# gddickinson/neural_enhanced_super_resolution

Measured on AMD Instinct MI355X. Metric: output megapixels/sec, RealESRGAN_x2plus x2 upscale, higher is better.
Workload: dtype f32 (operands as f16 hi+lo pairs, 3 f16 MFMAs per product, f32 accumulate); 1 GPU; c2: 512x512->1024x1024 RealESRGAN_x2plus fp32 single tile; frames_in_flight_per_gpu=1, world_size=1, partition=independent frames, no data-path collective

## Files before the change

### neural_enhanced_super_resolution_amd/csrc/conv3x3_f16x2.hip

```cpp
#include <cstdlib>
#include <type_traits>

#include "f16x2_common.h"
#include "nesr_kernels.h"

namespace nesr {


namespace {

constexpr int TW = 32, PW = TW + 2;
constexpr int WAVES = 4;
constexpr int RW = 2;

template <int DMAW>
struct Geo {
    static constexpr int LAUNCH_THREADS = 64 * (WAVES + DMAW);
    static constexpr int THREADS = 64 * (DMAW ? DMAW : WAVES);
    static constexpr int TH = WAVES * RW;
    static constexpr int PH = TH + 2;
    static constexpr int NPIX = PH * PW;
    static constexpr int IN_ITEMS = 4 * NPIX;
    static constexpr int IN_ROUNDS = (IN_ITEMS + THREADS - 1) / THREADS;
    static constexpr int IN_BYTES = IN_ITEMS * 16;
// ... 226 lines not shown
            for (int e = 0; e < 16; ++e) sum += acc16[r][e & 1][(e >> 1) & 1][(e >> 2) & 1][e & 3];
        if (sum == 12345.678f) static_cast<float*>(a.out)[0] = sum;
        return;
    }

    const int cb = cb16;
    const uint16_t* res1 = static_cast<const uint16_t*>(a.res1);
    const uint16_t* res2 = static_cast<const uint16_t*>(a.res2);
    uint16_t* out = static_cast<uint16_t*>(a.out);
    uint16_t* out2 = static_cast<uint16_t*>(a.out2);
    bool bad = false;
    const bool poison = a.cout_real > 0 && a.status && __builtin_nontemporal_load(a.status) != 0u;
#pragma unroll
    for (int r = 0; r < RW; ++r)
#pragma unroll
        for (int nh = 0; nh < 2; ++nh) {
            const int Y = y0 + RW * wave + r, X = x0 + 16 * nh + j16;
            const bool valid = X < a.w_ && Y < y_hi;
            const size_t pix = ((size_t)n * a.h + (Y < a.h ? Y : 0)) * a.w_ + (X < a.w_ ? X : 0);
            f32x4 v0, v1;
#pragma unroll
            for (int i = 0; i < 4; ++i) {
                const float e = fmaf(acc16[r][nh][0][1][i], LO_INV, acc16[r][nh][0][0][i]);
                const float o = fmaf(acc16[r][nh][1][1][i], LO_INV, acc16[r][nh][1][0][i]);
                const auto sw_ = __builtin_amdgcn_permlane16_swap(__float_as_uint(e), __float_as_uint(o), false, false);
                v0[i] = __uint_as_float(sw_[0]);
                v1[i] = __uint_as_float(sw_[1]);
            }
            v0 += bz0;
            v1 += bz1;
            if (a.lrelu) {
#pragma unroll
                for (int i = 0; i < 4; ++i) { v0[i] = fmaxf(v0[i], v0[i] * 0.2f); v1[i] = fmaxf(v1[i], v1[i] * 0.2f); }
            }
            auto slot = [&](const Map& mp, int coff) -> size_t { return (size_t)((coff + 32 * cg) >> 4) * mp.chunk + pix * mp.pix + piece8; };
            if (res1) {
                f32x4 q0, q1;
                load_regrouped(res1 + slot(a.res1_map, 0), a.res1_map.chunk, q0, q1);
#pragma unroll
                for (int i = 0; i < 4; ++i) { v0[i] = __fadd_rn(__fmul_rn(v0[i], a.s1), q0[i]); v1[i] = __fadd_rn(__fmul_rn(v1[i], a.s1), q1[i]); }
            }
            if (res2) {
                f32x4 q0, q1;
                load_regrouped(res2 + slot(a.res2_map, 0), a.res2_map.chunk, q0, q1);
#pragma unroll
                for (int i = 0; i < 4; ++i) { v0[i] = __fadd_rn(__fmul_rn(v0[i], a.s2), q0[i]); v1[i] = __fadd_rn(__fmul_rn(v1[i], a.s2), q1[i]); }
            }
            if (out || out2) {
                uint4 cx, cx1;
                bool bad_here = false;
                split_regroup(v0, v1, cx, cx1, bad_here);
                bad |= bad_here && valid;
                if (valid && out) {
                    uint16_t* p = out + slot(a.out_map, a.out_coff);
                    store16(p, cx);
                    store16(p + a.out_map.chunk, cx1);
                }
                if (valid && out2) {
                    uint16_t* p = out2 + slot(a.out2_map, 0);
                    store16(p, cx);
                    store16(p + a.out2_map.chunk, cx1);
                }
            }
            if (!valid) continue;
            if (a.cout_real > 0 && cb == 0) {
#pragma unroll
                for (int q = 0; q < 4; ++q) {
                    if (q >= a.cout_real) break;
                    const float x = poison ? __builtin_nanf("") : v0[q];
                    if (a.out_nchw) a.out_nchw[(((size_t)n * a.cout_real + q) * a.h + Y) * a.w_ + X] = x;
                    if (a.out_u8) {
                        float qv = fminf(fmaxf(x, 0.f), 1.f) * 255.0f;
                        qv = a.u8_round ? rintf(qv) : truncf(qv);
                        const int ch = a.u8_flip ? (a.cout_real - 1 - q) : q;
                        a.out_u8[pix * a.cout_real + ch] = (uint8_t)qv;
                    }
                }
            }
        }
    if (bad && a.status) __hip_atomic_store(a.status, 1u, __ATOMIC_RELAXED, __HIP_MEMORY_SCOPE_AGENT);
    STAMP(3);
#if NESR_ABL & 64
    asm volatile("s_waitcnt vmcnt(0)" ::: "memory");
    STAMP(4);
#endif
}

struct RdbArgs {
    const void* cur;
    long long chunk_bytes;
    void* out;
    const void* res2;
    float s1, s2;
    const void* w[5];
    const float* bias[5];
    int n, h, w_;
    unsigned* progress;
    unsigned epoch;
    unsigned* abort_flag;
    unsigned* status;
    unsigned long long timeout_ticks;
};

__device__ __forceinline__ void glds16_s_sc1(const char* sbase, unsigned voff, unsigned lds_dst) {
    unsigned keep;
    asm volatile(
        "s_mov_b32 %0, m0\n\t"
        "s_mov_b32 m0, %3\n\t"
        "s_nop 0\n\t"
        "global_load_lds_dwordx4 %1, %2 sc1\n\t"
        "s_mov_b32 m0, %0"
        : "=&s"(keep)
        : "v"(voff), "s"(sbase), "s"(lds_dst)
        : "memory");
}
__device__ __forceinline__ void store16_wt_s(const char* sbase, unsigned voff, uint4 v) {
    asm volatile("global_store_dwordx4 %0, %1, %2 sc1\n\ts_nop 1" ::"v"(voff), "v"(__builtin_bit_cast(f32x4, v)), "s"(sbase) : "memory");
}

#ifndef NESR_RDB_ABL
#define NESR_RDB_ABL 0
#endif

__device__ __forceinline__ void wait_vmcnt_le(int k) {
    switch (k) {
        case 0: asm volatile("s_waitcnt vmcnt(0)" ::: "memory"); break;
        case 1: asm volatile("s_waitcnt vmcnt(1)" ::: "memory"); break;
        case 2: asm volatile("s_waitcnt vmcnt(2)" ::: "memory"); break;
        case 3: asm volatile("s_waitcnt vmcnt(3)" ::: "memory"); break;
        case 4: asm volatile("s_waitcnt vmcnt(4)" ::: "memory"); break;
        case 5: asm volatile("s_waitcnt vmcnt(5)" ::: "memory"); break;
        case 6: asm volatile("s_waitcnt vmcnt(6)" ::: "memory"); break;
        case 7: asm volatile("s_waitcnt vmcnt(7)" ::: "memory"); break;
        case 8: asm volatile("s_waitcnt vmcnt(8)" ::: "memory"); break;
        case 9: asm volatile("s_waitcnt vmcnt(9)" ::: "memory"); break;
        case 10: asm volatile("s_waitcnt vmcnt(10)" ::: "memory"); break;
        case 11: asm volatile("s_waitcnt vmcnt(11)" ::: "memory"); break;
        default: asm volatile("s_waitcnt vmcnt(12)" ::: "memory"); break;
    }
}

#if NESR_RDB_ABL & 256
__device__ unsigned long long g_rdb_stamps[2][64][8];
__device__ unsigned long long g_rdb_taps[2][8][8];
__device__ unsigned long long g_rdb_arrive[12][8][2];
#define RARRIVE(w, step, ev) do { if (blockIdx.x == 77 && lane == 0 && (step) >= 20 && (step) < 28) { unsigned long long t_ = __builtin_amdgcn_s_memtime(); asm volatile("s_waitcnt lgkmcnt(0)" ::: "memory"); g_rdb_arrive[w][(step) - 20][ev] = t_; } } while (0)
#define RSTAMP(role, step, ev) do { if (blockIdx.x == 77 && lane == 0) { unsigned long long t_ = __builtin_amdgcn_s_memtime(); asm volatile("s_waitcnt lgkmcnt(0)" ::: "memory"); g_rdb_stamps[role][step][ev] = t_; } } while (0)
#else
#define RSTAMP(role, step, ev) do { } while (0)
#define RARRIVE(w, step, ev) do { } while (0)
#endif

constexpr int RSLOTS = 4;
constexpr int MW = 8;
constexpr int DW = 4;
#ifndef NESR_RDB_PAR
#define NESR_RDB_PAR 0
#endif
#ifndef NESR_RDB_EPI_STEPS
#define NESR_RDB_EPI_STEPS 1
#endif
constexpr int EPI_STEPS = NESR_RDB_EPI_STEPS;
static_assert(EPI_STEPS <= 4 - (RSLOTS - 1), "the tile would wait for its own progress word");

__global__ __launch_bounds__(64 * (MW + DW), 3) void rdb_f16x2_kernel(RdbArgs a) {
    typedef Geo<4> G;
    constexpr int THREADS = G::THREADS, TH = G::TH;
    constexpr int IN_ITEMS = G::IN_ITEMS, IN_ROUNDS = G::IN_ROUNDS, IN_BYTES = G::IN_BYTES;
    constexpr int W_ROUNDS = (W_ITEMS + THREADS - 1) / THREADS;
    constexpr int WRING = RSLOTS * IN_BYTES;
    constexpr int BIAS = RSLOTS * (IN_BYTES + W_BYTES);
    static_assert(TH == MW, "one tile row per MFMA wave");
    extern __shared__ __attribute__((aligned(16))) char smem[];

    const int lane = threadIdx.x & 63;
    const int wave_all = __builtin_amdgcn_readfirstlane(threadIdx.x >> 6);
    const bool is_dma = wave_all >= MW;
    const bool is_cmp = !is_dma;
    const int wave = is_cmp ? wave_all : wave_all - MW;
    const int tid = wave * 64 + lane;

    const int tiles_x = (a.w_ + TW - 1) / TW;
    const int tiles_y = (a.h + TH - 1) / TH;
    const int total = tiles_x * tiles_y * a.n;
    int tile;
    {
        const int bid = blockIdx.x, q = total >> 3, r = total & 7, xcd = bid & 7;
        tile = (xcd < r ? xcd * (q + 1) : r * (q + 1) + (xcd - r) * q) + (bid >> 3);
    }
    const int n = tile / (tiles_x * tiles_y);
    const int t2 = tile - n * tiles_x * tiles_y;
    const int ty = t2 / tiles_x, tx = t2 - ty * tiles_x;
    const int y0 = ty * TH, x0 = tx * TW;

    const int j16 = lane & 15, g4 = lane >> 4;
    auto advance = [](int& l, int& cg, int& c) {
        const int nc = l == 4 ? 12 : 4 + 2 * l, ncg = l == 4 ? 2 : 1;
        if (++c == nc) { c = 0; if (++cg == ncg) { cg = 0; ++l; } }
    };

    if (is_dma) {
#ifdef NESR_RDB_DMAPRIO
        __builtin_amdgcn_s_setprio(NESR_RDB_DMAPRIO);
#endif
        const unsigned lds_base = (unsigned)(size_t)(lds_char*)(smem);
        unsigned voff[IN_ROUNDS];
        unsigned okmask = 0;
        unsigned wavemask = 0;
        const int row0 = y0 > 0 ? y0 - 1 : 0;
        const char* in_img = static_cast<const char*>(a.cur) + ((size_t)n * a.h + row0) * a.w_ * 64;
        const unsigned* watch = nullptr;
        int kdma = 0;
        if (lane < 9) {
            const int ny = ty + lane / 3 - 1, nx = tx + lane % 3 - 1;
            if (ny >= 0 && ny < tiles_y && nx >= 0 && nx < tiles_x) watch = a.progress + (n * tiles_y + ny) * tiles_x + nx;
        }
        {
            int p = tid >> 2;
            int py = p / PW, px = p - py * PW;
            const int sl = tid & 3;
#pragma unroll
            for (int i = 0; i < IN_ROUNDS; ++i) {
                const int k = tid + THREADS * i;
                const int sg = sl ^ (((px >> 2) & 1) << 1);
                const int Y = y0 - 1 + py, X = x0 - 1 + px;
                const bool has = k < IN_ITEMS;
                const bool ok = has && Y >= 0 && Y < a.h && X >= 0 && X < a.w_;
                voff[i] = ((unsigned)(Y - row0) * (unsigned)a.w_ + (unsigned)X) * 64u + sg * 16;
                okmask |= ok ? (1u << i) : 0u;
                if (__builtin_amdgcn_ballot_w64(ok) != 0ull) { wavemask |= 1u << i; ++kdma; }
                if (has && !ok) {
#pragma unroll
                    for (int sl2 = 0; sl2 < RSLOTS; ++sl2) *reinterpret_cast<f32x4*>(smem + sl2 * IN_BYTES + k * 16) = f32x4{0.f, 0.f, 0.f, 0.f};
                }
                px += (THREADS / 4) % PW;
                py += (THREADS / 4) / PW;
                if (px >= PW) { px -= PW; py += 1; }
            }
#pragma unroll
            for (int j = 0; j < W_ROUNDS; ++j) kdma += (wave * 64 + THREADS * j) < W_ITEMS ? 1 : 0;
        }
        unsigned seen = 0;
        bool gave_up = __hip_atomic_load(a.abort_flag, __ATOMIC_RELAXED, __HIP_MEMORY_SCOPE_AGENT) != 0u;
        auto dma_step = [&](int l, int cg, int c, int slot) {
            const int CG = l == 4 ? 2 : 1;
            const char* wsrc = static_cast<const char*>(a.w[l]) + ((size_t)c * CG + cg) * W_BYTES;
#pragma unroll
            for (int j = 0; j < W_ROUNDS; ++j) {
                const int k = tid + THREADS * j;
                const unsigned dst = lds_base + WRING + slot * W_BYTES + j * (THREADS * 16) + wave * 1024;
                if (k < W_ITEMS && !(NESR_RDB_ABL & 64)) glds16_s(wsrc, (unsigned)k * 16u, __builtin_amdgcn_readfirstlane(dst));
            }
            const unsigned need = c < 4 ? 0u : (unsigned)((c - 4) >> 1) + 1u;
            if (need > seen && !gave_up && !(NESR_RDB_ABL & 1)) {
                const unsigned target = a.epoch + need;
                unsigned long long t0 = 0;
                for (unsigned it = 0;; ++it) {
                    const unsigned v = watch ? __hip_atomic_load(watch, __ATOMIC_RELAXED, __HIP_MEMORY_SCOPE_AGENT) : target;
                    if (__builtin_amdgcn_ballot_w64((int)(v - target) < 0) == 0ull) break;
                    if ((it & 63u) == 0u) {
                        const unsigned long long now = __builtin_amdgcn_s_memrealtime();
                        if (it == 0) t0 = now;
                        const unsigned ab = __hip_atomic_load(a.abort_flag, __ATOMIC_RELAXED, __HIP_MEMORY_SCOPE_AGENT);
                        if (ab != 0u || now - t0 > a.timeout_ticks) {
                            if (ab == 0u && lane == 0) __hip_atomic_store(a.abort_flag, 1u | ((unsigned)c << 8) | ((unsigned)tile << 16), __ATOMIC_RELAXED, __HIP_MEMORY_SCOPE_AGENT);
                            gave_up = true;
                            break;
                        }
                    }
                    __builtin_amdgcn_s_sleep(4);
                }
                seen = need;
            }
            const char* isrc = in_img + (long long)c * a.chunk_bytes;
#pragma unroll
            for (int i = 0; i < IN_ROUNDS; ++i) {
                const unsigned dst = lds_base + slot * IN_BYTES + i * (THREADS * 16) + wave * 1024;
                if (((wavemask >> i) & 1u) && !(NESR_RDB_ABL & 32)) {
                    if ((okmask >> i) & 1u) {
                        if (NESR_RDB_ABL & 2) glds16_s(isrc, voff[i], __builtin_amdgcn_readfirstlane(dst));
                        else glds16_s_sc1(isrc, voff[i], __builtin_amdgcn_readfirstlane(dst));
                    }
                }
            }
        };
        if (wave == 0 && lane < 48) {
            const int l = lane >> 3 > 4 ? 4 : lane >> 3, cgq = lane >> 3 > 4 ? 8 + (lane & 7) : (lane & 7);
            *reinterpret_cast<f32x4*>(smem + BIAS + lane * 16) = *reinterpret_cast<const f32x4*>(a.bias[l] + 4 * cgq);
        }
        int fl = 0, fcg = 0, fc = 0;
        dma_step(0, 0, 0, 0);
        advance(fl, fcg, fc);
        dma_step(fl, fcg, fc, 1);
        advance(fl, fcg, fc);
        dma_step(fl, fcg, fc, 2);
        advance(fl, fcg, fc);
        asm volatile("s_waitcnt lgkmcnt(0)" ::: "memory");
        int fill = 3;
        int cl = 0, ccg = 0, cc = 0;
        wait_vmcnt_le((NESR_RDB_ABL & 96) ? 0 : 2 * kdma);
        __builtin_amdgcn_s_barrier();
        asm volatile("" ::: "memory");
        for (int step = 0; step < 52; ++step) {
            if (wave == 0) RSTAMP(1, step, 0);
#if NESR_RDB_ABL & 256
            if ((step == 0 || step == 51) && wave == 0 && blockIdx.x == 77 && lane == 0) {
                const unsigned long long r_ = __builtin_amdgcn_s_memrealtime(), t_ = __builtin_amdgcn_s_memtime();
                asm volatile("s_waitcnt lgkmcnt(0)" ::: "memory");
                g_rdb_stamps[1][step == 0 ? 62 : 63][0] = r_;
                g_rdb_stamps[1][step == 0 ? 62 : 63][1] = t_;
            }
#endif
            wait_vmcnt_le((step >= 50 || (NESR_RDB_ABL & 96)) ? 0 : kdma);
            if (wave == 0) RSTAMP(1, step, 1);
            RARRIVE(MW + wave, step, 0);
            if (!(NESR_RDB_ABL & 512)) __builtin_amdgcn_s_barrier();
            asm volatile("" ::: "memory");
            RARRIVE(MW + wave, step, 1);
            if (wave == 0) RSTAMP(1, step, 2);
            if (cc == EPI_STEPS && ccg == 0 && cl >= 1 && wave == 0 && lane == 0)
                __hip_atomic_store(a.progress + tile, a.epoch + (unsigned)cl, __ATOMIC_RELAXED, __HIP_MEMORY_SCOPE_AGENT);
            if (fl < 5) {
                dma_step(fl, fcg, fc, fill);
                advance(fl, fcg, fc);
                fill = fill == RSLOTS - 1 ? 0 : fill + 1;
            }
            if (wave == 0) RSTAMP(1, step, 3);
            advance(cl, ccg, cc);
        }
        return;
    }

#ifdef NESR_RDB_YPRIO
    if (wave >= 4) __builtin_amdgcn_s_setprio(NESR_RDB_YPRIO);
#endif
    const bool active = (y0 + wave) < a.h;
    const int un = g4 >> 1, kh = g4 & 1;
    int b16[5][2], a16[5];
#pragma unroll
    for (int st_ = 0; st_ < 5; ++st_) {
        const int dy = st_ < 3 ? un : 2;
        const int dx = st_ < 3 ? st_ : (st_ == 3 ? un : 2);
#pragma unroll
        for (int nh = 0; nh < 2; ++nh) {
            const int col = 16 * nh + j16 + dx;
            b16[st_][nh] = ((wave + dy) * PW + col) * 64 + ((kh ^ (((col >> 2) & 1) << 1)) << 4);
        }
        a16[st_] = ((((dy * 3 + dx) * 2) * 2 + kh) * 32 + j16) * 16;
    }
    int slot = 0;
#if NESR_RDB_ABL & 256
    int mstep = 0;
#endif
    typedef const __attribute__((address_space(3))) f32x4* lds_f32x4;
    const unsigned lds0 = (unsigned)(size_t)(lds_char*)(smem);
    unsigned bcur[5][2], acur[5], acur4b;
#pragma unroll
    for (int t = 0; t < 5; ++t) {
        bcur[t][0] = lds0 + (unsigned)b16[t][0];
        bcur[t][1] = lds0 + (unsigned)(t == 4 ? (b16[4][0] ^ ((un ^ 1) << 5)) : (b16[t][0] ^ 32));
        acur[t] = lds0 + (unsigned)(WRING + a16[t]);
    }
    acur4b = acur[4] + (unsigned)un * 1024u;
    const int par = (NESR_RDB_PAR >= 0) ? NESR_RDB_PAR : wave >> 2;
    const int cbl = (g4 & 1) * 16 + (g4 >> 1) * 8;
    const int piece8 = ((g4 & 1) * 2 + (g4 >> 1)) * 8;
    const bool res2 = a.res2 != nullptr;
    f32x4 ep[2][2];
#pragma unroll
    for (int nh = 0; nh < 2; ++nh)
#pragma unroll
        for (int mt = 0; mt < 2; ++mt) ep[nh][mt] = f32x4{0.f, 0.f, 0.f, 0.f};
    int ep_l = -1, ep_cg = 0;
    bool bad = false;
    auto unpack_res = [&](f32x4 rx, f32x4 rx1, f32x4& q0, f32x4& q1) {
        uint4 cx = __builtin_bit_cast(uint4, rx), cx1 = __builtin_bit_cast(uint4, rx1);
        regroup_pairs(cx, cx1);
        const f16x8 h = __builtin_bit_cast(f16x8, cx), lo = __builtin_bit_cast(f16x8, cx1);
#pragma unroll
        for (int i = 0; i < 4; ++i) {
            q0[i] = fmaf((float)lo[i], LO_INV, (float)h[i]);
            q1[i] = fmaf((float)lo[4 + i], LO_INV, (float)h[4 + i]);
        }
    };
    const long long row_bytes = (((long long)n * a.h + (y0 + wave)) * a.w_) * 64;
    unsigned lane_off[2];
    bool lane_ok[2];
#pragma unroll
    for (int nh = 0; nh < 2; ++nh) {
        const int X = x0 + 16 * nh + j16;
        lane_ok[nh] = X < a.w_;
        lane_off[nh] = (unsigned)(lane_ok[nh] ? X : 0) * 64u + (unsigned)piece8 * 2u;
    }
    auto uni = [](const char* p) -> const char* {
        const unsigned long long v = (unsigned long long)p;
        const unsigned lo = __builtin_amdgcn_readfirstlane((unsigned)v), hi = __builtin_amdgcn_readfirstlane((unsigned)(v >> 32));
        return (const char*)(((unsigned long long)hi << 32) | lo);
    };
    auto epi_half = [&](int l, int cg, const f32x4& e0, const f32x4& e1, int nh) {
#if NESR_RDB_ABL & 256
        if (wave == 1) RSTAMP(0, mstep, 3);
#endif
        const bool valid = lane_ok[nh];
        const unsigned voff = lane_off[nh];
        const char* bsrc = smem + BIAS + (l * 32 + 32 * cg + cbl) * 4;
        f32x4 v0, v1;
#pragma unroll
        for (int i = 0; i < 4; ++i) {
            const auto sw_ = __builtin_amdgcn_permlane16_swap(__float_as_uint(e0[i]), __float_as_uint(e1[i]), false, false);
            v0[i] = __uint_as_float(sw_[0]);
            v1[i] = __uint_as_float(sw_[1]);
        }
        v0 += *reinterpret_cast<const f32x4*>(bsrc);
        v1 += *reinterpret_cast<const f32x4*>(bsrc + 16);
        const int dchunk = l == 4 ? 2 * cg : 4 + 2 * l;
        if (l < 4) {
#pragma unroll
            for (int i = 0; i < 4; ++i) { v0[i] = fmaxf(v0[i], v0[i] * 0.2f); v1[i] = fmaxf(v1[i], v1[i] * 0.2f); }
        } else {
            const char* r1 = uni(static_cast<const char*>(a.cur) + (long long)(2 * cg) * a.chunk_bytes + row_bytes);
            const f32x4 r10 = *reinterpret_cast<const f32x4*>(r1 + voff), r11 = *reinterpret_cast<const f32x4*>(r1 + a.chunk_bytes + voff);
            f32x4 r20 = r10, r21 = r11;
            if (res2) {
                const char* r2 = uni(static_cast<const char*>(a.res2) + (long long)(2 * cg) * a.chunk_bytes + row_bytes);
                r20 = *reinterpret_cast<const f32x4*>(r2 + voff);
                r21 = *reinterpret_cast<const f32x4*>(r2 + a.chunk_bytes + voff);
            }
            f32x4 q0, q1;
            unpack_res(r10, r11, q0, q1);
#pragma unroll
            for (int i = 0; i < 4; ++i) { v0[i] = __fadd_rn(__fmul_rn(v0[i], a.s1), q0[i]); v1[i] = __fadd_rn(__fmul_rn(v1[i], a.s1), q1[i]); }
            if (res2) {
                unpack_res(r20, r21, q0, q1);
#pragma unroll
                for (int i = 0; i < 4; ++i) { v0[i] = __fadd_rn(__fmul_rn(v0[i], a.s2), q0[i]); v1[i] = __fadd_rn(__fmul_rn(v1[i], a.s2), q1[i]); }
            }
        }
#if NESR_RDB_ABL & 256
        asm volatile("" :: "v"(v0), "v"(v1));
        if (wave == 1) RSTAMP(0, mstep, 4);
#endif
        uint4 cx, cx1;
        bool bad_here = false;
        split_regroup(v0, v1, cx, cx1, bad_here);
        bad |= bad_here && valid;
#if NESR_RDB_ABL & 256
        asm volatile("" :: "v"(__builtin_bit_cast(f32x4, cx)), "v"(__builtin_bit_cast(f32x4, cx1)));
        if (wave == 1) RSTAMP(0, mstep, 5);
#endif
        if (valid) {
            const char* d0 = uni(static_cast<const char*>(l == 4 ? a.out : a.cur) + (long long)dchunk * a.chunk_bytes + row_bytes);
            if (l < 4 && !(NESR_RDB_ABL & 4)) {
                store16_wt_s(d0, voff, cx);
                store16_wt_s(d0 + a.chunk_bytes, voff, cx1);
            } else {
                *reinterpret_cast<uint4*>(const_cast<char*>(d0) + voff) = cx;
                *reinterpret_cast<uint4*>(const_cast<char*>(d0) + a.chunk_bytes + voff) = cx1;
            }
        }
#if NESR_RDB_ABL & 256
        if (wave == 1) RSTAMP(0, mstep, 6);
#endif
    };
    auto epi_part = [&](int c) {
        if (NESR_RDB_ABL & 16) return;
        if (EPI_STEPS == 1) {
            epi_half(ep_l, ep_cg, ep[0][0], ep[0][1], 0);
            epi_half(ep_l, ep_cg, ep[1][0], ep[1][1], 1);
        } else if (c == 0) {
            epi_half(ep_l, ep_cg, ep[0][0], ep[0][1], 0);
        } else {
            epi_half(ep_l, ep_cg, ep[1][0], ep[1][1], 1);
        }
    };
    f32x4 acc16[2][2][2];
    f32x4 Af[2][2][2];
    f32x4 Bf[2][2][2];
    auto load_step = [&](int sl, int s_, int buf) {
        const bool wrap = sl == RSLOTS - 1;
        const unsigned dB = wrap ? (unsigned)(-(RSLOTS - 1) * IN_BYTES) : (unsigned)IN_BYTES;
        const unsigned dA = wrap ? (unsigned)(-(RSLOTS - 1) * W_BYTES) : (unsigned)W_BYTES;
#pragma unroll
        for (int mt = 0; mt < 2; ++mt) {
            if (s_ < 4) {
                Af[buf][mt][0] = *((lds_f32x4)(size_t)(acur[s_] + mt * 256));
                Af[buf][mt][1] = *((lds_f32x4)(size_t)(acur[s_] + mt * 256 + 1024));
            } else {
                f32x4 hi = *((lds_f32x4)(size_t)(acur[4] + mt * 256));
                Af[buf][mt][1] = *((lds_f32x4)(size_t)(acur4b + mt * 256));
                if (un) hi = f32x4{0.f, 0.f, 0.f, 0.f};
                Af[buf][mt][0] = hi;
            }
        }
#pragma unroll
        for (int nh = 0; nh < 2; ++nh) {
            Bf[buf][nh][0] = *((lds_f32x4)(size_t)(bcur[s_][0] + nh * 1024));
            Bf[buf][nh][1] = *((lds_f32x4)(size_t)(bcur[s_][1] + nh * 1024));
        }
        acur[s_] += dA;
        if (s_ == 4) acur4b += dA;
        bcur[s_][0] += dB;
        bcur[s_][1] += dB;
    };
    auto step_body = [&](auto Pc, int c, bool last_of_all) {
        constexpr int P = decltype(Pc)::value;
        if (c == EPI_STEPS) asm volatile("s_waitcnt vmcnt(0)" ::: "memory");
#if NESR_RDB_ABL & 256
        if (wave == 1) RSTAMP(0, mstep, 0);
        RARRIVE(wave, mstep, 0);
#endif
        if (!(NESR_RDB_ABL & 512)) __builtin_amdgcn_s_barrier();
        asm volatile("" ::: "memory");
#if NESR_RDB_ABL & 256
        RARRIVE(wave, mstep, 1);
        if (wave == 1) RSTAMP(0, mstep, 1);
#endif
        const bool epi_now = active && ep_l >= 0 && c < EPI_STEPS;
        const int nslot = slot == RSLOTS - 1 ? 0 : slot + 1;
        if (active && !(NESR_RDB_ABL & 8)) {
            if (epi_now && par == 0) {
                epi_part(c);
                __builtin_amdgcn_sched_barrier(0);
            }
#if NESR_RDB_ABL & 256
            unsigned long long tt[6];
#endif
#pragma unroll
            for (int s_ = 0; s_ < 5; ++s_) {
                const int buf = (s_ + P) & 1;
#if NESR_RDB_ABL & 256
                tt[s_] = __builtin_amdgcn_s_memtime();
                __builtin_amdgcn_sched_barrier(0);
#endif
                if (s_ + 1 < 5) load_step(slot, s_ + 1, buf ^ 1);
                else if (!last_of_all) load_step(nslot, 0, buf ^ 1);
#pragma unroll
                for (int mt = 0; mt < 2; ++mt) {
                    const f16x8 a0 = __builtin_bit_cast(f16x8, Af[buf][mt][0]), a1 = __builtin_bit_cast(f16x8, Af[buf][mt][1]);
#pragma unroll
                    for (int nh = 0; nh < 2; ++nh) {
                        const f16x8 x0_ = __builtin_bit_cast(f16x8, Bf[buf][nh][0]), x1_ = __builtin_bit_cast(f16x8, Bf[buf][nh][1]);
                        if (s_ < 4) {
                            acc16[nh][mt][1] = __builtin_amdgcn_mfma_f32_16x16x32_f16(a0, x1_, acc16[nh][mt][1], 0, 0, 0);
                            acc16[nh][mt][0] = __builtin_amdgcn_mfma_f32_16x16x32_f16(a0, x0_, acc16[nh][mt][0], 0, 0, 0);
                            acc16[nh][mt][1] = __builtin_amdgcn_mfma_f32_16x16x32_f16(a1, x0_, acc16[nh][mt][1], 0, 0, 0);
                        } else {
                            acc16[nh][mt][0] = __builtin_amdgcn_mfma_f32_16x16x32_f16(a0, x0_, acc16[nh][mt][0], 0, 0, 0);
                            acc16[nh][mt][1] = __builtin_amdgcn_mfma_f32_16x16x32_f16(a1, x1_, acc16[nh][mt][1], 0, 0, 0);
                        }
                    }
                }
#pragma unroll
                for (int i = 0; i < 8; ++i) {
                    __builtin_amdgcn_sched_group_barrier(0x008, 1, 0);
                    __builtin_amdgcn_sched_group_barrier(0x100, 1, 0);
                }
                __builtin_amdgcn_sched_barrier(0);
            }
            if (epi_now && par == 1) {
                epi_part(c);
                __builtin_amdgcn_sched_barrier(0);
            }
#if NESR_RDB_ABL & 256
            tt[5] = __builtin_amdgcn_s_memtime();
            if (blockIdx.x == 77 && (wave == 1 || wave == 5) && lane == 0 && mstep >= 20 && mstep < 28) {
#pragma unroll
                for (int i = 0; i < 6; ++i) g_rdb_taps[wave == 5][mstep - 20][i] = tt[i];
            }
#endif
        }
        slot = nslot;
#if NESR_RDB_ABL & 256
        if (wave == 1) RSTAMP(0, mstep, 2);
        ++mstep;
#endif
    };
    __builtin_amdgcn_s_barrier();
    asm volatile("" ::: "memory");
    if (active) load_step(0, 0, 0);
    for (int l = 0; l < 5; ++l) {
        const int nc = l == 4 ? 12 : 4 + 2 * l;
        const int ncg = l == 4 ? 2 : 1;
        for (int cg = 0; cg < ncg; ++cg) {
#pragma unroll
            for (int nh = 0; nh < 2; ++nh)
#pragma unroll
                for (int mt = 0; mt < 2; ++mt)
#pragma unroll
                    for (int q = 0; q < 2; ++q) acc16[nh][mt][q] = f32x4{0.f, 0.f, 0.f, 0.f};
            for (int c = 0; c < nc; c += 2) {
                step_body(std::integral_constant<int, 0>{}, c, false);
                step_body(std::integral_constant<int, 1>{}, c + 1, l == 4 && cg == 1 && c + 2 == nc);
            }
#pragma unroll
            for (int nh = 0; nh < 2; ++nh)
#pragma unroll
                for (int mt = 0; mt < 2; ++mt)
#pragma unroll
                    for (int i = 0; i < 4; ++i) ep[nh][mt][i] = fmaf(acc16[nh][mt][1][i], LO_INV, acc16[nh][mt][0][i]);
            ep_l = l;
            ep_cg = cg;
        }
    }
    if (active && !(NESR_RDB_ABL & 16)) {
        epi_half(4, 1, ep[0][0], ep[0][1], 0);
        epi_half(4, 1, ep[1][0], ep[1][1], 1);
    }
    if (bad && a.status) __hip_atomic_store(a.status, 1u, __ATOMIC_RELAXED, __HIP_MEMORY_SCOPE_AGENT);
}

template <int DMAW, int NMT = 2>
hipError_t launch_split(const ConvArgs& a, hipStream_t s) {
    typedef Geo<DMAW> G;
    constexpr size_t shm = (size_t)ISLOTS * G::IN_BYTES + 2 * (size_t)W_BYTES;
    static unsigned long long attr_done = 0;
    {
        const hipError_t e = ensure_dynamic_lds(reinterpret_cast<const void*>(&conv3x3_f16x2_kernel<DMAW, NMT>), shm, attr_done);
        if (e != hipSuccess) return e;
    }
    const int rows = (a.y_hi > 0 ? a.y_hi : a.h) - a.y_lo;
    const long total = (long)((a.w_ + TW - 1) / TW) * ((rows + G::TH - 1) / G::TH) * a.n * (a.coutp / 32);
    if (total <= 0) return hipSuccess;
    if (total > 0x7fffffffL) return hipErrorInvalidValue;
    hipLaunchKernelGGL((conv3x3_f16x2_kernel<DMAW, NMT>), dim3((unsigned)total), dim3(G::LAUNCH_THREADS), shm, s, a);
    return hipGetLastError();
}


}

#if NESR_RDB_ABL & 256
extern "C" int nesr_debug_rdb_stamps(unsigned long long* out) {
    return (int)hipMemcpyFromSymbol(out, HIP_SYMBOL(g_rdb_stamps), sizeof(unsigned long long) * 2 * 64 * 8);
}
extern "C" int nesr_debug_rdb_taps(unsigned long long* out) {
    return (int)hipMemcpyFromSymbol(out, HIP_SYMBOL(g_rdb_taps), sizeof(unsigned long long) * 2 * 8 * 8);
}
extern "C" int nesr_debug_rdb_arrive(unsigned long long* out) {
    return (int)hipMemcpyFromSymbol(out, HIP_SYMBOL(g_rdb_arrive), sizeof(unsigned long long) * 12 * 8 * 2);
}
#endif
#if NESR_ABL & 64
extern "C" int nesr_debug_stamps(unsigned long long* out, int n) {
    return (int)hipMemcpyFromSymbol(out, HIP_SYMBOL(g_stamps), sizeof(unsigned long long) * (n < 256 ? n : 256));
}
#endif

size_t packed_weight_elems_f16x2(int cin_p, int coutp) { return (size_t)cin_p * 9 * coutp * 2; }

void pack_weights_f16x2(const float* oihw, int cout, int cin, int cin_p, int coutp, uint16_t* dst) {
    const size_t total = packed_weight_elems_f16x2(cin_p, coutp);
    for (size_t i = 0; i < total; ++i) dst[i] = 0;
    const int groups = coutp / 32;
    for (int o = 0; o < cout; ++o)
        for (int ci = 0; ci < cin; ++ci)
            for (int tap = 0; tap < 9; ++tap) {
                const float wv = oihw[((size_t)o * cin + ci) * 9 + tap];
                const uint16_t hi = f2h(wv);
                const uint16_t lo = f2h((wv - h2f(hi)) * LO_SCALE);
                const int c = ci / 16, kh = (ci % 16) / 8, kk = ci % 8;
                const size_t slab = ((size_t)c * groups + o / 32) * (size_t)(W_ITEMS * 8);
                const size_t ihi = slab + ((((size_t)tap * 2 + 0) * 2 + kh) * 32 + o % 32) * 8 + kk;
                const size_t ilo = slab + ((((size_t)tap * 2 + 1) * 2 + kh) * 32 + o % 32) * 8 + kk;
                dst[ihi] = hi;
                dst[ilo] = lo;
            }
}

int rdb_f16x2_tiles(int n, int h, int w) { return ((w + TW - 1) / TW) * ((h + 7) / 8) * n; }

hipError_t launch_rdb_f16x2(const RdbLaunch& r, hipStream_t s) {
    typedef Geo<4> G;
    constexpr size_t shm = (size_t)RSLOTS * (G::IN_BYTES + (size_t)W_BYTES) + 768;
    static unsigned long long attr_done = 0;
    {
        const hipError_t e = ensure_dynamic_lds(reinterpret_cast<const void*>(&rdb_f16x2_kernel), shm, attr_done);
        if (e != hipSuccess) return e;
    }
    if ((long long)r.w_ * 64 * 12 >= (1ll << 32)) return hipErrorInvalidValue;
    RdbArgs a;
    a.cur = r.cur; a.chunk_bytes = r.chunk_bytes; a.out = r.out; a.res2 = r.res2; a.s1 = r.s1; a.s2 = r.s2;
    for (int i = 0; i < 5; ++i) { a.w[i] = r.w[i]; a.bias[i] = r.bias[i]; }
    a.n = r.n; a.h = r.h; a.w_ = r.w_;
    a.progress = r.progress; a.epoch = r.epoch; a.abort_flag = r.abort_flag; a.status = r.status;
    a.timeout_ticks = r.timeout_ticks ? r.timeout_ticks : 20000000ull;
    int total = rdb_f16x2_tiles(r.n, r.h, r.w_);
    if (total <= 0) return hipSuccess;
    static int resident = -1;
    if (resident < 0) {
        int per_cu = 0, dev = 0, cus = 0;
        if (hipOccupancyMaxActiveBlocksPerMultiprocessor(&per_cu, rdb_f16x2_kernel, 64 * (MW + DW), shm) != hipSuccess || hipGetDevice(&dev) != hipSuccess ||
            hipDeviceGetAttribute(&cus, hipDeviceAttributeMultiprocessorCount, dev) != hipSuccess)
            return hipErrorUnknown;
        resident = per_cu * cus;
    }
    if (total > resident) return hipErrorLaunchOutOfResources;
    total -= r.debug_drop;
    if (total <= 0) return hipSuccess;
    hipLaunchKernelGGL(rdb_f16x2_kernel, dim3((unsigned)total), dim3(64 * (MW + DW)), shm, s, a);
    return hipGetLastError();
}

hipError_t launch_conv3x3_f16x2(const ConvArgs& a, hipStream_t s) {
    if (a.cin % 16 || (a.coutp != 32 && a.coutp != 64)) return hipErrorInvalidValue;
    if (a.y_lo < 0 || (a.y_hi > 0 && (a.y_hi > a.h || a.y_hi <= a.y_lo)) || (a.y_hi == 0 && a.y_lo != 0)) return hipErrorInvalidValue;
    if ((long long)a.in_w * 64 * 12 >= (1ll << 32)) return hipErrorInvalidValue;
    if (a.in_map.pix != 32 || (a.out && (a.out_map.pix % 32 || a.out_coff % 16))) return hipErrorInvalidValue;
    if ((a.out_nchw || a.out_u8) && (a.coutp != 32 || a.cout_real < 1 || a.cout_real > 4)) return hipErrorInvalidValue;
    static const int cus = [] {
        int dev = 0, n = 256;
        if (hipGetDevice(&dev) != hipSuccess || hipDeviceGetAttribute(&n, hipDeviceAttributeMultiprocessorCount, dev) != hipSuccess) n = 256;
        return n;
    }();
    static const int dmaw = [] { const char* e = getenv("NESR_SPLIT_DMAW"); return e ? atoi(e) : -1; }();
    const long t1 = (long)((a.w_ + TW - 1) / TW) * (((a.y_hi > 0 ? a.y_hi : a.h) - a.y_lo + 7) / 8) * a.n * (a.coutp >> 5);
    const bool producer = dmaw >= 0 ? dmaw > 0 : (t1 <= cus && !a.shared_device);
    if (a.narrow_last && (a.out_nchw || a.out_u8) && !a.out && !a.out2 && !a.res1 && !a.res2)
        return producer ? launch_split<4, 1>(a, s) : launch_split<0, 1>(a, s);
    return producer ? launch_split<4>(a, s) : launch_split<0>(a, s);
}

}
```

Baseline: 159.7 MP/s.

## Fuse conv5's two output-channel groups into one pass over shared input slabs

Inside the fused RDB kernel, the fifth conv no longer runs its two 32-channel output groups as separate sweeps. Each input slab is now loaded once and feeds two accumulator sets, so the conv5 steps go from 24 to 12. The weight DMA is split from the input DMA: conv5 weight pairs are streamed into ring positions 0,1 / 2,3, and the vmcnt wait tracks the real number of in-flight loads. This removes half the input LDS reads and DMA steps for conv5, but doubles the accumulator registers, which may lower occupancy or cause spills under launch bounds of 3.

Result: faster. 168.4 MP/s (median of 6 runs) (+5.5%).

```diff
diff --git a/neural_enhanced_super_resolution_amd/csrc/conv3x3_f16x2.hip b/neural_enhanced_super_resolution_amd/csrc/conv3x3_f16x2.hip
--- a/neural_enhanced_super_resolution_amd/csrc/conv3x3_f16x2.hip
+++ b/neural_enhanced_super_resolution_amd/csrc/conv3x3_f16x2.hip
@@ -402,6 +402,10 @@
 #endif
 
 constexpr int RSLOTS = 4;
+constexpr int RDB_STEP5 = 4 + 6 + 8 + 10;
+constexpr int RDB_STEPS = RDB_STEP5 + 12;
+constexpr int W5_ROUNDS = 2 * W_ITEMS / (64 * 4);
+static_assert(RSLOTS == 4 && RDB_STEP5 % RSLOTS == 0 && W5_ROUNDS * 64 * 4 == 2 * W_ITEMS, "conv5's slab pairs sit at ring positions 0,1 / 2,3 and fill whole DMA rounds");
 constexpr int MW = 8;
 constexpr int DW = 4;
 #ifndef NESR_RDB_PAR
@@ -444,9 +448,9 @@
     const int y0 = ty * TH, x0 = tx * TW;
 
     const int j16 = lane & 15, g4 = lane >> 4;
-    auto advance = [](int& l, int& cg, int& c) {
-        const int nc = l == 4 ? 12 : 4 + 2 * l, ncg = l == 4 ? 2 : 1;
-        if (++c == nc) { c = 0; if (++cg == ncg) { cg = 0; ++l; } }
+    auto advance = [](int& l, int& c) {
+        const int nc = l == 4 ? 12 : 4 + 2 * l;
+        if (++c == nc) { c = 0; ++l; }
     };
 
     if (is_dma) {
@@ -460,7 +464,7 @@
         const int row0 = y0 > 0 ? y0 - 1 : 0;
         const char* in_img = static_cast<const char*>(a.cur) + ((size_t)n * a.h + row0) * a.w_ * 64;
         const unsigned* watch = nullptr;
-        int kdma = 0;
+        int kin = 0, kw = 0;
         if (lane < 9) {
             const int ny = ty + lane / 3 - 1, nx = tx + lane % 3 - 1;
             if (ny >= 0 && ny < tiles_y && nx >= 0 && nx < tiles_x) watch = a.progress + (n * tiles_y + ny) * tiles_x + nx;
@@ -478,7 +482,7 @@
                 const bool ok = has && Y >= 0 && Y < a.h && X >= 0 && X < a.w_;
                 voff[i] = ((unsigned)(Y - row0) * (unsigned)a.w_ + (unsigned)X) * 64u + sg * 16;
                 okmask |= ok ? (1u << i) : 0u;
-                if (__builtin_amdgcn_ballot_w64(ok) != 0ull) { wavemask |= 1u << i; ++kdma; }
+                if (__builtin_amdgcn_ballot_w64(ok) != 0ull) { wavemask |= 1u << i; ++kin; }
                 if (has && !ok) {
 #pragma unroll
                     for (int sl2 = 0; sl2 < RSLOTS; ++sl2) *reinterpret_cast<f32x4*>(smem + sl2 * IN_BYTES + k * 16) = f32x4{0.f, 0.f, 0.f, 0.f};
@@ -488,19 +492,28 @@
                 if (px >= PW) { px -= PW; py += 1; }
             }
 #pragma unroll
-            for (int j = 0; j < W_ROUNDS; ++j) kdma += (wave * 64 + THREADS * j) < W_ITEMS ? 1 : 0;
+            for (int j = 0; j < W_ROUNDS; ++j) kw += (wave * 64 + THREADS * j) < W_ITEMS ? 1 : 0;
         }
         unsigned seen = 0;
         bool gave_up = __hip_atomic_load(a.abort_flag, __ATOMIC_RELAXED, __HIP_MEMORY_SCOPE_AGENT) != 0u;
-        auto dma_step = [&](int l, int cg, int c, int slot) {
-            const int CG = l == 4 ? 2 : 1;
-            const char* wsrc = static_cast<const char*>(a.w[l]) + ((size_t)c * CG + cg) * W_BYTES;
+        auto dma_w = [&](int l, int c, int wpos) {
+            const char* wsrc = static_cast<const char*>(a.w[l]) + (size_t)c * W_BYTES;
 #pragma unroll
             for (int j = 0; j < W_ROUNDS; ++j) {
                 const int k = tid + THREADS * j;
-                const unsigned dst = lds_base + WRING + slot * W_BYTES + j * (THREADS * 16) + wave * 1024;
+                const unsigned dst = lds_base + WRING + wpos * W_BYTES + j * (THREADS * 16) + wave * 1024;
                 if (k < W_ITEMS && !(NESR_RDB_ABL & 64)) glds16_s(wsrc, (unsigned)k * 16u, __builtin_amdgcn_readfirstlane(dst));
             }
+        };
+        auto dma_w5 = [&](int c, int wpos) {
+            const char* wsrc = static_cast<const char*>(a.w[4]) + (size_t)c * (2 * W_BYTES);
+#pragma unroll
+            for (int j = 0; j < W5_ROUNDS; ++j) {
+                const unsigned dst = lds_base + WRING + wpos * W_BYTES + j * (THREADS * 16) + wave * 1024;
+                if (!(NESR_RDB_ABL & 64)) glds16_s(wsrc, (unsigned)(tid + THREADS * j) * 16u, __builtin_amdgcn_readfirstlane(dst));
+            }
+        };
+        auto dma_in = [&](int c, int slot) {
             const unsigned need = c < 4 ? 0u : (unsigned)((c - 4) >> 1) + 1u;
             if (need > seen && !gave_up && !(NESR_RDB_ABL & 1)) {
                 const unsigned target = a.epoch + need;
@@ -538,45 +551,54 @@
             const int l = lane >> 3 > 4 ? 4 : lane >> 3, cgq = lane >> 3 > 4 ? 8 + (lane & 7) : (lane & 7);
             *reinterpret_cast<f32x4*>(smem + BIAS + lane * 16) = *reinterpret_cast<const f32x4*>(a.bias[l] + 4 * cgq);
         }
-        int fl = 0, fcg = 0, fc = 0;
-        dma_step(0, 0, 0, 0);
-        advance(fl, fcg, fc);
-        dma_step(fl, fcg, fc, 1);
-        advance(fl, fcg, fc);
-        dma_step(fl, fcg, fc, 2);
-        advance(fl, fcg, fc);
+        int fl = 0, fc = 0;
+#pragma unroll
+        for (int i = 0; i < RSLOTS - 1; ++i) {
+            dma_w(0, i, i);
+            dma_in(i, i);
+            advance(fl, fc);
+        }
         asm volatile("s_waitcnt lgkmcnt(0)" ::: "memory");
         int fill = 3;
-        int cl = 0, ccg = 0, cc = 0;
-        wait_vmcnt_le((NESR_RDB_ABL & 96) ? 0 : 2 * kdma);
+        int cl = 0, cc = 0;
+        wait_vmcnt_le((NESR_RDB_ABL & 96) ? 0 : 2 * (kw + kin));
+        int inflight = kw + kin;
         __builtin_amdgcn_s_barrier();
         asm volatile("" ::: "memory");
-        for (int step = 0; step < 52; ++step) {
+        for (int step = 0; step < RDB_STEPS; ++step) {
             if (wave == 0) RSTAMP(1, step, 0);
 #if NESR_RDB_ABL & 256
-            if ((step == 0 || step == 51) && wave == 0 && blockIdx.x == 77 && lane == 0) {
+            if ((step == 0 || step == RDB_STEPS - 1) && wave == 0 && blockIdx.x == 77 && lane == 0) {
                 const unsigned long long r_ = __builtin_amdgcn_s_memrealtime(), t_ = __builtin_amdgcn_s_memtime();
                 asm volatile("s_waitcnt lgkmcnt(0)" ::: "memory");
                 g_rdb_stamps[1][step == 0 ? 62 : 63][0] = r_;
                 g_rdb_stamps[1][step == 0 ? 62 : 63][1] = t_;
             }
 #endif
-            wait_vmcnt_le((step >= 50 || (NESR_RDB_ABL & 96)) ? 0 : kdma);
+            wait_vmcnt_le((NESR_RDB_ABL & 96) ? 0 : inflight);
             if (wave == 0) RSTAMP(1, step, 1);
             RARRIVE(MW + wave, step, 0);
             if (!(NESR_RDB_ABL & 512)) __builtin_amdgcn_s_barrier();
             asm volatile("" ::: "memory");
             RARRIVE(MW + wave, step, 1);
             if (wave == 0) RSTAMP(1, step, 2);
-            if (cc == EPI_STEPS && ccg == 0 && cl >= 1 && wave == 0 && lane == 0)
+            if (cc == EPI_STEPS && cl >= 1 && wave == 0 && lane == 0)
                 __hip_atomic_store(a.progress + tile, a.epoch + (unsigned)cl, __ATOMIC_RELAXED, __HIP_MEMORY_SCOPE_AGENT);
+            inflight = 0;
+            if (step + 1 >= RDB_STEP5) {
+                if (step + 1 < RDB_STEPS) dma_w5(step + 1 - RDB_STEP5, ((step + 1) & 1) * 2);
+            } else if (fl < 4) {
+                dma_w(fl, fc, (step + RSLOTS - 1) & (RSLOTS - 1));
+                inflight += kw;
+            }
             if (fl < 5) {
-                dma_step(fl, fcg, fc, fill);
-                advance(fl, fcg, fc);
+                dma_in(fc, fill);
+                inflight += kin;
+                advance(fl, fc);
                 fill = fill == RSLOTS - 1 ? 0 : fill + 1;
             }
             if (wave == 0) RSTAMP(1, step, 3);
-            advance(cl, ccg, cc);
+            advance(cl, cc);
         }
         return;
     }
@@ -599,19 +621,20 @@
         a16[st_] = ((((dy * 3 + dx) * 2) * 2 + kh) * 32 + j16) * 16;
     }
     int slot = 0;
+    int wpos = 0;
 #if NESR_RDB_ABL & 256
     int mstep = 0;
 #endif
     typedef const __attribute__((address_space(3))) f32x4* lds_f32x4;
     const unsigned lds0 = (unsigned)(size_t)(lds_char*)(smem);
-    unsigned bcur[5][2], acur[5], acur4b;
-#pragma unroll
-    for (int t = 0; t < 5; ++t) {
-        bcur[t][0] = lds0 + (unsigned)b16[t][0];
-        bcur[t][1] = lds0 + (unsigned)(t == 4 ? (b16[4][0] ^ ((un ^ 1) << 5)) : (b16[t][0] ^ 32));
-        acur[t] = lds0 + (unsigned)(WRING + a16[t]);
-    }
-    acur4b = acur[4] + (unsigned)un * 1024u;
+    unsigned bcur[5], aw012, aw3, aw4, aw4b;
+#pragma unroll
+    for (int t = 0; t < 5; ++t) bcur[t] = lds0 + (unsigned)b16[t][0];
+    const unsigned xl4 = (unsigned)((un ^ 1) << 5);
+    aw012 = lds0 + (unsigned)(WRING + a16[0]);
+    aw3 = lds0 + (unsigned)(WRING + a16[3]);
+    aw4 = lds0 + (unsigned)(WRING + a16[4]);
+    aw4b = aw4 + (unsigned)un * 1024u;
     const int par = (NESR_RDB_PAR >= 0) ? NESR_RDB_PAR : wave >> 2;
     const int cbl = (g4 & 1) * 16 + (g4 >> 1) * 8;
     const int piece8 = ((g4 & 1) * 2 + (g4 >> 1)) * 8;
@@ -621,7 +644,7 @@
     for (int nh = 0; nh < 2; ++nh)
 #pragma unroll
         for (int mt = 0; mt < 2; ++mt) ep[nh][mt] = f32x4{0.f, 0.f, 0.f, 0.f};
-    int ep_l = -1, ep_cg = 0;
+    int ep_l = -1;
     bool bad = false;
     auto unpack_res = [&](f32x4 rx, f32x4 rx1, f32x4& q0, f32x4& q1) {
         uint4 cx = __builtin_bit_cast(uint4, rx), cx1 = __builtin_bit_cast(uint4, rx1);
@@ -715,44 +738,75 @@
     auto epi_part = [&](int c) {
         if (NESR_RDB_ABL & 16) return;
         if (EPI_STEPS == 1) {
-            epi_half(ep_l, ep_cg, ep[0][0], ep[0][1], 0);
-            epi_half(ep_l, ep_cg, ep[1][0], ep[1][1], 1);
+            epi_half(ep_l, 0, ep[0][0], ep[0][1], 0);
+            epi_half(ep_l, 0, ep[1][0], ep[1][1], 1);
         } else if (c == 0) {
-            epi_half(ep_l, ep_cg, ep[0][0], ep[0][1], 0);
+            epi_half(ep_l, 0, ep[0][0], ep[0][1], 0);
         } else {
-            epi_half(ep_l, ep_cg, ep[1][0], ep[1][1], 1);
-        }
-    };
-    f32x4 acc16[2][2][2];
+            epi_half(ep_l, 0, ep[1][0], ep[1][1], 1);
+        }
+    };
+    f32x4 acc16[2][2][2][2];
     f32x4 Af[2][2][2];
     f32x4 Bf[2][2][2];
-    auto load_step = [&](int sl, int s_, int buf) {
-        const bool wrap = sl == RSLOTS - 1;
-        const unsigned dB = wrap ? (unsigned)(-(RSLOTS - 1) * IN_BYTES) : (unsigned)IN_BYTES;
-        const unsigned dA = wrap ? (unsigned)(-(RSLOTS - 1) * W_BYTES) : (unsigned)W_BYTES;
+    auto load_a = [&](int s_, int buf, unsigned off) {
 #pragma unroll
         for (int mt = 0; mt < 2; ++mt) {
             if (s_ < 4) {
-                Af[buf][mt][0] = *((lds_f32x4)(size_t)(acur[s_] + mt * 256));
-                Af[buf][mt][1] = *((lds_f32x4)(size_t)(acur[s_] + mt * 256 + 1024));
+                const unsigned ad = s_ < 3 ? aw012 + s_ * 2048 : aw3;
+                Af[buf][mt][0] = *((lds_f32x4)(size_t)(ad + off + mt * 256));
+                Af[buf][mt][1] = *((lds_f32x4)(size_t)(ad + off + mt * 256 + 1024));
             } else {
-                f32x4 hi = *((lds_f32x4)(size_t)(acur[4] + mt * 256));
-                Af[buf][mt][1] = *((lds_f32x4)(size_t)(acur4b + mt * 256));
+                f32x4 hi = *((lds_f32x4)(size_t)(aw4 + off + mt * 256));
+                Af[buf][mt][1] = *((lds_f32x4)(size_t)(aw4b + off + mt * 256));
                 if (un) hi = f32x4{0.f, 0.f, 0.f, 0.f};
                 Af[buf][mt][0] = hi;
             }
         }
+    };
+    auto move_a = [&](unsigned d) {
+        aw012 += d;
+        aw3 += d;
+        aw4 += d;
+        aw4b += d;
+    };
+    auto load_b = [&](int sl, int s_, int buf) {
+        const unsigned dB = sl == RSLOTS - 1 ? (unsigned)(-(RSLOTS - 1) * IN_BYTES) : (unsigned)IN_BYTES;
+        const unsigned xl = bcur[s_] ^ (s_ == 4 ? xl4 : 32u);
 #pragma unroll
         for (int nh = 0; nh < 2; ++nh) {
-            Bf[buf][nh][0] = *((lds_f32x4)(size_t)(bcur[s_][0] + nh * 1024));
-            Bf[buf][nh][1] = *((lds_f32x4)(size_t)(bcur[s_][1] + nh * 1024));
-        }
-        acur[s_] += dA;
-        if (s_ == 4) acur4b += dA;
-        bcur[s_][0] += dB;
-        bcur[s_][1] += dB;
-    };
-    auto step_body = [&](auto Pc, int c, bool last_of_all) {
+            Bf[buf][nh][0] = *((lds_f32x4)(size_t)(bcur[s_] + nh * 1024));
+            Bf[buf][nh][1] = *((lds_f32x4)(size_t)(xl + nh * 1024));
+        }
+        bcur[s_] += dB;
+    };
+    auto mfma_tap = [&](int s_, int g, int abuf, int bbuf) {
+#pragma unroll
+        for (int mt = 0; mt < 2; ++mt) {
+            const f16x8 a0 = __builtin_bit_cast(f16x8, Af[abuf][mt][0]), a1 = __builtin_bit_cast(f16x8, Af[abuf][mt][1]);
+#pragma unroll
+            for (int nh = 0; nh < 2; ++nh) {
+                const f16x8 x0_ = __builtin_bit_cast(f16x8, Bf[bbuf][nh][0]), x1_ = __builtin_bit_cast(f16x8, Bf[bbuf][nh][1]);
+                if (s_ < 4) {
+                    acc16[g][nh][mt][1] = __builtin_amdgcn_mfma_f32_16x16x32_f16(a0, x1_, acc16[g][nh][mt][1], 0, 0, 0);
+                    acc16[g][nh][mt][0] = __builtin_amdgcn_mfma_f32_16x16x32_f16(a0, x0_, acc16[g][nh][mt][0], 0, 0, 0);
+                    acc16[g][nh][mt][1] = __builtin_amdgcn_mfma_f32_16x16x32_f16(a1, x0_, acc16[g][nh][mt][1], 0, 0, 0);
+                } else {
+                    acc16[g][nh][mt][0] = __builtin_amdgcn_mfma_f32_16x16x32_f16(a0, x0_, acc16[g][nh][mt][0], 0, 0, 0);
+                    acc16[g][nh][mt][1] = __builtin_amdgcn_mfma_f32_16x16x32_f16(a1, x1_, acc16[g][nh][mt][1], 0, 0, 0);
+                }
+            }
+        }
+    };
+    auto zero_acc = [&](int g) {
+#pragma unroll
+        for (int nh = 0; nh < 2; ++nh)
+#pragma unroll
+            for (int mt = 0; mt < 2; ++mt)
+#pragma unroll
+                for (int q = 0; q < 2; ++q) acc16[g][nh][mt][q] = f32x4{0.f, 0.f, 0.f, 0.f};
+    };
+    auto step_body = [&](auto Pc, int c) {
         constexpr int P = decltype(Pc)::value;
         if (c == EPI_STEPS) asm volatile("s_waitcnt vmcnt(0)" ::: "memory");
 #if NESR_RDB_ABL & 256
@@ -767,6 +821,7 @@
 #endif
         const bool epi_now = active && ep_l >= 0 && c < EPI_STEPS;
         const int nslot = slot == RSLOTS - 1 ? 0 : slot + 1;
+        const unsigned dA = wpos == RSLOTS - 1 ? (unsigned)(-(RSLOTS - 1) * W_BYTES) : (unsigned)W_BYTES;
         if (active && !(NESR_RDB_ABL & 8)) {
             if (epi_now && par == 0) {
                 epi_part(c);
@@ -782,24 +837,14 @@
                 tt[s_] = __builtin_amdgcn_s_memtime();
                 __builtin_amdgcn_sched_barrier(0);
 #endif
-                if (s_ + 1 < 5) load_step(slot, s_ + 1, buf ^ 1);
-                else if (!last_of_all) load_step(nslot, 0, buf ^ 1);
-#pragma unroll
-                for (int mt = 0; mt < 2; ++mt) {
-                    const f16x8 a0 = __builtin_bit_cast(f16x8, Af[buf][mt][0]), a1 = __builtin_bit_cast(f16x8, Af[buf][mt][1]);
-#pragma unroll
-                    for (int nh = 0; nh < 2; ++nh) {
-                        const f16x8 x0_ = __builtin_bit_cast(f16x8, Bf[buf][nh][0]), x1_ = __builtin_bit_cast(f16x8, Bf[buf][nh][1]);
-                        if (s_ < 4) {
-                            acc16[nh][mt][1] = __builtin_amdgcn_mfma_f32_16x16x32_f16(a0, x1_, acc16[nh][mt][1], 0, 0, 0);
-                            acc16[nh][mt][0] = __builtin_amdgcn_mfma_f32_16x16x32_f16(a0, x0_, acc16[nh][mt][0], 0, 0, 0);
-                            acc16[nh][mt][1] = __builtin_amdgcn_mfma_f32_16x16x32_f16(a1, x0_, acc16[nh][mt][1], 0, 0, 0);
-                        } else {
-                            acc16[nh][mt][0] = __builtin_amdgcn_mfma_f32_16x16x32_f16(a0, x0_, acc16[nh][mt][0], 0, 0, 0);
-                            acc16[nh][mt][1] = __builtin_amdgcn_mfma_f32_16x16x32_f16(a1, x1_, acc16[nh][mt][1], 0, 0, 0);
-                        }
-                    }
-                }
+                if (s_ + 1 < 5) {
+                    load_a(s_ + 1, buf ^ 1, 0);
+                    load_b(slot, s_ + 1, buf ^ 1);
+                } else {
+                    load_a(0, buf ^ 1, dA);
+                    load_b(nslot, 0, buf ^ 1);
+                }
+                mfma_tap(s_, 0, buf, buf);
 #pragma unroll
                 for (int i = 0; i < 8; ++i) {
                     __builtin_amdgcn_sched_group_barrier(0x008, 1, 0);
@@ -819,42 +864,117 @@
             }
 #endif
         }
+        move_a(dA);
         slot = nslot;
+        wpos = wpos == RSLOTS - 1 ? 0 : wpos + 1;
 #if NESR_RDB_ABL & 256
         if (wave == 1) RSTAMP(0, mstep, 2);
         ++mstep;
 #endif
     };
+    auto step_body5 = [&](auto Pc, auto Fc, int c, bool last_of_all) {
+        constexpr int P = decltype(Pc)::value;
+        constexpr bool FIRST = decltype(Fc)::value != 0;
+        if (c == EPI_STEPS) asm volatile("s_waitcnt vmcnt(0)" ::: "memory");
+#if NESR_RDB_ABL & 256
+        if (wave == 1) RSTAMP(0, mstep, 0);
+        RARRIVE(wave, mstep, 0);
+#endif
+        if (!(NESR_RDB_ABL & 512)) __builtin_amdgcn_s_barrier();
+        asm volatile("" ::: "memory");
+#if NESR_RDB_ABL & 256
+        RARRIVE(wave, mstep, 1);
+        if (wave == 1) RSTAMP(0, mstep, 1);
+#endif
+        const bool epi_now = active && ep_l >= 0 && c < EPI_STEPS;
+        const int nslot = slot == RSLOTS - 1 ? 0 : slot + 1;
+        const unsigned dA = wpos == 0 ? (unsigned)(2 * W_BYTES) : (unsigned)(-2 * W_BYTES);
+        if (active && !(NESR_RDB_ABL & 8)) {
+            load_a(0, 0, 0);
+            if (epi_now && par == 0) {
+                epi_part(c);
+                __builtin_amdgcn_sched_barrier(0);
+            }
+            if (FIRST) { zero_acc(0); zero_acc(1); }
+#pragma unroll
+            for (int s_ = 0; s_ < 5; ++s_) {
+                const int buf = (s_ + P) & 1;
+                load_a(s_, 1, W_BYTES);
+                if (s_ + 1 < 5) load_b(slot, s_ + 1, buf ^ 1);
+                else if (!last_of_all) load_b(nslot, 0, buf ^ 1);
+                mfma_tap(s_, 0, 0, buf);
+#pragma unroll
+                for (int i = 0; i < 8; ++i) {
+                    __builtin_amdgcn_sched_group_barrier(0x008, 1, 0);
+                    __builtin_amdgcn_sched_group_barrier(0x100, 1, 0);
+                }
+                __builtin_amdgcn_sched_barrier(0);
+                if (s_ + 1 < 5) load_a(s_ + 1, 0, 0);
+                mfma_tap(s_, 1, 1, buf);
+                if (s_ + 1 < 5) {
+#pragma unroll
+                    for (int i = 0; i < 4; ++i) {
+                        __builtin_amdgcn_sched_group_barrier(0x008, 2, 0);
+                        __builtin_amdgcn_sched_group_barrier(0x100, 1, 0);
+                    }
+                }
+                __builtin_amdgcn_sched_barrier(0);
+            }
+            if (epi_now && par == 1) {
+                epi_part(c);
+                __builtin_amdgcn_sched_barrier(0);
+            }
+        }
+        move_a(dA);
+        slot = nslot;
+        wpos = wpos == 0 ? 2 : 0;
+#if NESR_RDB_ABL & 256
+        if (wave == 1) RSTAMP(0, mstep, 2);
+        ++mstep;
+#endif
+    };
     __builtin_amdgcn_s_barrier();
     asm volatile("" ::: "memory");
-    if (active) load_step(0, 0, 0);
-    for (int l = 0; l < 5; ++l) {
-        const int nc = l == 4 ? 12 : 4 + 2 * l;
-        const int ncg = l == 4 ? 2 : 1;
-        for (int cg = 0; cg < ncg; ++cg) {
-#pragma unroll
-            for (int nh = 0; nh < 2; ++nh)
-#pragma unroll
-                for (int mt = 0; mt < 2; ++mt)
-#pragma unroll
-                    for (int q = 0; q < 2; ++q) acc16[nh][mt][q] = f32x4{0.f, 0.f, 0.f, 0.f};
-            for (int c = 0; c < nc; c += 2) {
-                step_body(std::integral_constant<int, 0>{}, c, false);
-                step_body(std::integral_constant<int, 1>{}, c + 1, l == 4 && cg == 1 && c + 2 == nc);
-            }
-#pragma unroll
-            for (int nh = 0; nh < 2; ++nh)
-#pragma unroll
-                for (int mt = 0; mt < 2; ++mt)
-#pragma unroll
-                    for (int i = 0; i < 4; ++i) ep[nh][mt][i] = fmaf(acc16[nh][mt][1][i], LO_INV, acc16[nh][mt][0][i]);
-            ep_l = l;
-            ep_cg = cg;
-        }
+    if (active) {
+        load_a(0, 0, 0);
+        load_b(0, 0, 0);
+    }
+    typedef std::integral_constant<int, 0> I0;
+    typedef std::integral_constant<int, 1> I1;
+    for (int l = 0; l < 4; ++l) {
+        const int nc = 4 + 2 * l;
+        zero_acc(0);
+        for (int c = 0; c < nc; c += 2) {
+            step_body(I0{}, c);
+            step_body(I1{}, c + 1);
+        }
+#pragma unroll
+        for (int nh = 0; nh < 2; ++nh)
+#pragma unroll
+            for (int mt = 0; mt < 2; ++mt)
+#pragma unroll
+                for (int i = 0; i < 4; ++i) ep[nh][mt][i] = fmaf(acc16[0][nh][mt][1][i], LO_INV, acc16[0][nh][mt][0][i]);
+        ep_l = l;
+    }
+    step_body5(I0{}, I1{}, 0, false);
+    step_body5(I1{}, I0{}, 1, false);
+    for (int c = 2; c < 12; c += 2) {
+        step_body5(I0{}, I0{}, c, false);
+        step_body5(I1{}, I0{}, c + 1, c + 2 == 12);
     }
     if (active && !(NESR_RDB_ABL & 16)) {
-        epi_half(4, 1, ep[0][0], ep[0][1], 0);
-        epi_half(4, 1, ep[1][0], ep[1][1], 1);
+#pragma unroll
+        for (int g = 0; g < 2; ++g)
+#pragma unroll
+            for (int nh = 0; nh < 2; ++nh) {
+                f32x4 e0, e1;
+#pragma unroll
+                for (int i = 0; i < 4; ++i) {
+                    e0[i] = fmaf(acc16[g][nh][0][1][i], LO_INV, acc16[g][nh][0][0][i]);
+                    e1[i] = fmaf(acc16[g][nh][1][1][i], LO_INV, acc16[g][nh][1][0][i]);
+                }
+                epi_half(4, g, e0, e1, nh);
+            }
     }
     if (bad && a.status) __hip_atomic_store(a.status, 1u, __ATOMIC_RELAXED, __HIP_MEMORY_SCOPE_AGENT);
 }
@@ -880,6 +1000,7 @@
 }
 
 #if NESR_RDB_ABL & 256
+extern "C" int nesr_debug_rdb_steps() { return RDB_STEPS; }
 extern "C" int nesr_debug_rdb_stamps(unsigned long long* out) {
     return (int)hipMemcpyFromSymbol(out, HIP_SYMBOL(g_rdb_stamps), sizeof(unsigned long long) * 2 * 64 * 8);
 }
```
